# SebLague/Ray-Tracing

Hardware: AMD Instinct MI355X
Metric: Mrays/s at 1920x1080, 8 spp, 8 bounces; per-channel L2 vs reference (higher is better)
Workload: dtype f32

## Files before the change

### ray-tracing_amd/csrc/rt_context.hip

```cpp
#include <hip/hip_runtime.h>

#include <math.h>
#include <stdarg.h>
#include <stdio.h>
#include <stdlib.h>
#include <string.h>
#include <dlfcn.h>
#include <sys/mman.h>

#include <cmath>
#include <string>
#include <vector>

#include <algorithm>
#include <chrono>
#include <mutex>

#include "rt_kernels.h"
#include "../../include/rt_cost.h"
#include "../../include/rt_primary.h"
#include "../../include/rt_tile_cand.h"
#include "../../include/rt_aov.h"
#include "../../include/rt_denoise.h"
#include "../../include/rt_reproject.h"
#include "../../include/rt_variance.h"
#include "../../include/rt_adaptive.h"
#include "../../include/rt_motion.h"
#include "../../include/rt_query.h"
#include "../../include/rt_radiance.h"

#include "rt_denoise_launch.h"
#include "rt_denoise_math.h"
#include "rt_reproject_launch.h"
#include "rt_variance_launch.h"
#include "rt_adaptive_launch.h"
#include "rt_query_launch.h"
#include "rt_radiance_launch.h"
#include "rt_layout.h"
#include "rt_launch_order.h"
#include "rt_launch_plan.h"
#include "rt_scene_prep.h"
#include "rt_primary.h"
#include "rt_tile_cand.h"
#define RT_VERSION_STRING "raytrace_hip gfx950 abi=1"

static thread_local char g_err[512] = "";

struct RtContext;
struct LaunchJob;
struct HipOrder final : rt_order::Backend {
    RtContext* ctx = nullptr;
    hipEvent_t ev[rt_order::EVENT_COUNT] = {};
    LaunchJob* job = nullptr;
    hipStream_t stream(int s) const;
    int record(rt_order::Event e, int s) override;
    int wait(int s, rt_order::Event e) override;
    int sort(int s, int target) override;
    int trace(int s, int part, int parts) override;
    int accumulate(int s) override;
};

struct RtContext {
    int device = 0;
    hipStream_t ownStream = nullptr;
    hipStream_t stream = nullptr;
    hipStream_t sideStream = nullptr;
// ... 25 lines not shown
    DChunk* dChunks = nullptr;
    int nChunks = 0, nFiltered = 0, extWords = 0;
    float filterMaxOrigin = 0.0f;
    std::vector<RtBVHNode> hRootChildren;
    std::vector<RtSphere> hSpheres;
    int nSpheres = 0, nModels = 0, nTris = 0, nPairs = 0;
    bool flatScene = false;
    int stackEntries = 1;
    int wavesPerGroup = 1;
    uint32_t hotUnits = 0;
    uint32_t poolSpinLimit = 1u << 16;
    int poolMinItems = 4;
    int poolWaves = 1, poolCells = 0;
    uint32_t travLimit = 1u << 20;
    bool haveScene = false;
    std::vector<RtModel> hModels;
    std::vector<uint32_t> hRootCodes;
    std::vector<int32_t> hTriBase;
    PrimaryTris primaryTris;
    bool primaryOn = true;
    int lastPrimaryOn = -1;
    bool tileCandOn = true;
    int lastTileCand = -1;
    uint32_t* dTileCand[2] = {nullptr, nullptr};
    int tileCandTiles = 0;
    bool tileCandValid[2] = {false, false};
    TileCandKey tileCandKey[2];
    bool tileCandWanted = false;
    TileCandKey tileCandWant;

    RtParams params;
    bool haveParams = false;
    int frame = 1;

    unsigned long long* dCounters = nullptr;
    unsigned long long* dTileQueue = nullptr;
    unsigned long long tileQueueNext[2] = {0, 0};
    uint32_t* dTileCost = nullptr;
    uint32_t* dTileOrder[2] = {nullptr, nullptr};
    uint32_t* dTileKey = nullptr;
    int orderTiles = 0;
    int numCUs = 256;
    int occPerCU[16] = {0};
    size_t occBytes[16] = {0};
    bool verbose = false;
    void* dPxCold = nullptr;
    long long pxColdWaves = 0;
    int frameGroupOverride = 0;
    bool coalesce = true;
    int pending = 0;
    bool fuseFrames = true;
    int fuseCap = RT_FUSE_MIN;
// ... 261 lines not shown
        ctx->numCUs = prop.multiProcessorCount;
        HIP_TRY(ctx, hipStreamCreateWithFlags(&ctx->ownStream, hipStreamNonBlocking));
        ctx->stream = ctx->ownStream;
        HIP_TRY(ctx, hipMalloc(&ctx->dCounters, sizeof(unsigned long long) * RT_COUNTER_SLOTS * RT_COUNTER_FIELDS));
        HIP_TRY(ctx, hipMemsetAsync(ctx->dCounters, 0, sizeof(unsigned long long) * RT_COUNTER_SLOTS * RT_COUNTER_FIELDS, ctx->ownStream));
        HIP_TRY(ctx, hipStreamCreateWithFlags(&ctx->sideStream, hipStreamNonBlocking));
        HIP_TRY(ctx, hipMalloc(&ctx->dTileQueue, 2 * sizeof(unsigned long long)));
        HIP_TRY(ctx, hipMemsetAsync(ctx->dTileQueue, 0, 2 * sizeof(unsigned long long), ctx->ownStream));
        HIP_TRY(ctx, hipStreamSynchronize(ctx->ownStream));
        HIP_TRY(ctx, hipEventCreate(&ctx->evStart));
        HIP_TRY(ctx, hipEventCreate(&ctx->evStop));
        for (hipEvent_t& ev : ctx->backend.ev) HIP_TRY(ctx, hipEventCreateWithFlags(&ev, hipEventDisableTiming));
        return RT_OK;
    };
    if (int rc = init()) {
        rt_destroy(ctx);
        return rc;
    }
    memset(&ctx->params, 0, sizeof(ctx->params));
    if (const char* g = getenv("RT_GRID")) ctx->gridOverride = atoi(g);
    if (const char* g = getenv("RT_POOL_MIN_ITEMS")) ctx->poolMinItems = atoi(g);
    if (const char* g = getenv("RT_PRIMARY")) ctx->primaryOn = atoi(g) != 0;
    if (const char* g = getenv("RT_TILE_CAND")) ctx->tileCandOn = atoi(g) != 0;
    if (const char* g = getenv("RT_POOL_FAULT")) { if (atoi(g)) ctx->poolSpinLimit = 64u | 0x80000000u; }
    if (getenv("RT_VERBOSE")) ctx->verbose = true;
    if (const char* f = getenv("RT_FUSE_FRAMES")) ctx->fuseFrames = atoi(f) != 0;
    if (const char* l = getenv("RT_LPT")) ctx->order.lpt = atoi(l) != 0;
    if (const char* t = getenv("RT_TWO_STREAMS")) ctx->twoStreams = atoi(t) != 0;
    if (const char* c = getenv("RT_COALESCE")) ctx->coalesce = atoi(c) != 0;
    if (const char* fg = getenv("RT_FRAME_GROUP")) ctx->frameGroupOverride = atoi(fg);
    if (const char* al = getenv("RT_ALTERNATE")) ctx->order.alternate = ctx->alternateWanted = atoi(al) != 0;
    ctx->order.set_two_streams(ctx->twoStreams && ctx->sideStream);
    if (const char* fc = getenv("RT_FUSE_CAP"))
        if (const int cap = rt_plan::pinned_fuse_cap(atoi(fc))) { ctx->fuseCap = cap; ctx->fuseCapPinned = true; }
    *out = ctx;
    return RT_OK;
}

static void free_scene(RtContext* ctx)
{
    hipFree(ctx->dSpheres); ctx->dSpheres = nullptr;
    hipFree(ctx->dMaterials); ctx->dMaterials = nullptr;
    hipFree(ctx->dModels); ctx->dModels = nullptr;
    hipFree(ctx->dPairs); ctx->dPairs = nullptr;
    hipFree(ctx->dTris); ctx->dTris = nullptr;
    hipFree(ctx->dNorms); ctx->dNorms = nullptr;
// ... 228 lines not shown
    if (!ps.lay.arena && (rc = commit_vec(ctx, &ctx->dTris, ps.lay.triBuf, peer ? &peer->dTris : nullptr, peer))) return rc;
    if ((rc = commit_vec(ctx, &ctx->dNorms, ps.lay.normBuf, peer ? &peer->dNorms : nullptr, peer))) return rc;
    if (ps.lay.unitTri.size() && (rc = commit_vec(ctx, &ctx->dUnitTri, ps.lay.unitTri, peer ? &peer->dUnitTri : nullptr, peer))) return rc;
    if ((rc = commit_vec(ctx, &ctx->dBigLeaves, ps.lay.bigLeaves, peer ? &peer->dBigLeaves : nullptr, peer))) return rc;
    ctx->arenaLayout = ps.lay.arena;
    ctx->layoutUsed = ps.lay.used.name();
    if ((rc = commit_vec(ctx, &ctx->dFilters, ps.filters, peer ? &peer->dFilters : nullptr, peer))) return rc;
    if ((rc = commit_vec(ctx, &ctx->dChunks, ps.chunks, peer ? &peer->dChunks : nullptr, peer))) return rc;
    ctx->nChunks = (int)ps.chunks.size();
    ctx->nFiltered = ps.nFiltered;
    ctx->extWords = ps.extWords;
    ctx->filterMaxOrigin = ps.maxOrigin;
    ctx->sphereBound = ps.sphereBound;
    ctx->hRootChildren = ps.rootChildren;
    ctx->hSpheres = ps.hSpheres;
    ctx->nSpheres = (int)ps.hSpheres.size();
    ctx->nModels = (int)ps.hModels.size();
    ctx->nTris = ps.nTris;
    ctx->nPairs = (int)ps.nPairs;
    ctx->hTriBase = ps.lay.triBase;
    {
        const auto& triSpace = ps.lay.arena ? ps.lay.pairBuf : ps.lay.triBuf;
        primary_collect_tris(ps.flat, ps.dmodels.data(), (int)ps.dmodels.size(), triSpace.data(), triSpace.size(), ps.lay.bigLeaves.data(), ps.lay.bigLeaves.size(), ctx->primaryTris);
    }
    ctx->stackEntries = ps.flat ? 0 : ps.maxHeight;
    ctx->flatScene = ps.flat;
    ctx->hotUnits = ps.flat ? 0u : ps.lay.hotUnits;
    {
        const unsigned long long steps = (unsigned long long)ps.hModels.size() * (2ull * ps.nPairs + 2ull) + 16ull;
        const unsigned long long lim = 2ull * 64ull * steps;
        ctx->travLimit = lim > 0x7fffffffull ? 0x7fffffffu : (uint32_t)lim;
        if (const char* e = getenv("RT_TRAV_LIMIT")) ctx->travLimit = (uint32_t)strtoul(e, nullptr, 10);
    }
    ctx->wavesPerGroup = ctx->hotUnits ? ps.wavesPerGroup : 1;
    {
        int on = 1, waves = RT_MAX_WAVES_PER_GROUP_FLAT;
        if (const char* e = getenv("RT_POOL")) on = atoi(e);
        if (const char* e = getenv("RT_POOL_WAVES")) waves = atoi(e);
        if (waves < 1) waves = 1;
        if (waves > RT_MAX_WAVES_PER_GROUP_FLAT) waves = RT_MAX_WAVES_PER_GROUP_FLAT;
        const bool pooled = ps.flat && on;
        ctx->poolWaves = pooled ? waves : 1;
        ctx->poolCells = pooled ? (int)RT_POOL_CELLS : 0;
    }
    ctx->hModels = ps.hModels;
    ctx->hRootCodes = ps.rootCodes;
// ... 224 lines not shown
    memcpy(a.dirToSun, p.dirToSun, 12);
    memcpy(a.viewParams, p.viewParams, 12);
    memcpy(a.cam, p.camLocalToWorld, 64);
    a.rcpWm1 = rt_rcp((float)a.W - 1.0f);
    a.rcpHm1 = rt_rcp((float)a.H - 1.0f);
    a.rcpW = rt_rcp((float)a.W);
    a.rcpSpp = rt_rcp((float)a.spp);
    {
        bool fin = true;
        for (int k = 0; k < 16; k++) fin = fin && std::isfinite(a.cam[k]);
        const rt_f3 o = primary_cam_origin(a.cam);
        const bool noNegZero = rt_f2u(o.x) != 0x80000000u && rt_f2u(o.y) != 0x80000000u && rt_f2u(o.z) != 0x80000000u;
        a.raygenNoDefocus = (a.defocus == 0.0f && fin && noNegZero && std::isfinite(a.rcpW)) ? 1 : 0;
        const bool allowed = withTable && ctx->haveScene &&
                             primary_allowed(ctx->primaryOn, a.raygenNoDefocus != 0, ctx->flatScene, ctx->nSpheres, ctx->nModels, ctx->primaryTris);
        std::vector<float> sph;
        DModel dm[RT_PRIMARY_MAX_MODELS];
        if (allowed) {
            float bound;
            pack_spheres(ctx->hSpheres.data(), ctx->nSpheres, sph, &bound);
            for (int i = 0; i < ctx->nModels; i++) pack_model(ctx->hModels[i], ctx->hRootCodes[i], ctx->hTriBase[i], dm[i]);
        }
        primary_fill(a.primary, allowed, o, sph.data(), ctx->nSpheres, ctx->sphereBound, dm, ctx->nModels, ctx->primaryTris);
        if (withTable) {
            ctx->lastPrimaryOn = a.primary.on;
            ctx->lastTileCand = 0;
            ctx->tileCandWanted = ctx->tileCandOn && a.primary.on != 0;
            if (ctx->tileCandWanted) {
                TileCandKey& k = ctx->tileCandWant;
                tile_cand_key_init(k);
                memcpy(k.cam, a.cam, sizeof(k.cam));
                memcpy(k.viewParams, a.viewParams, sizeof(k.viewParams));
                k.rcpWm1 = a.rcpWm1; k.rcpHm1 = a.rcpHm1; k.rcpW = a.rcpW; k.diverge = a.diverge;
                k.camOrigin[0] = o.x; k.camOrigin[1] = o.y; k.camOrigin[2] = o.z;
                k.W = (int32_t)a.W; k.H = (int32_t)a.H;
                k.tilesX = a.tilesX; k.tiles = a.tilesX * a.tilesY;
                k.stripRows = a.stripRows; k.partIndex = a.partIndex; k.partCount = a.partCount;
                k.nSpheres = ctx->nSpheres;
                memcpy(k.sph, sph.data(), sizeof(float) * 4 * (size_t)ctx->nSpheres);
            }
        }
    }
    a.counters = ctx->dCounters;
    a.travLimit = ctx->travLimit;
    a.poolSpinLimit = ctx->poolSpinLimit;
    a.wavesPerGroup = 1;
}

}

struct LaunchPlan {
// ... 77 lines not shown
        hipFree(ctx->dTileKey); ctx->dTileKey = nullptr;
        HIP_TRY(ctx, hipMalloc(&ctx->dTileCost, sizeof(uint32_t) * tiles));
        HIP_TRY(ctx, hipMalloc(&ctx->dTileOrder[0], sizeof(uint32_t) * tiles));
        HIP_TRY(ctx, hipMalloc(&ctx->dTileOrder[1], sizeof(uint32_t) * tiles));
        HIP_TRY(ctx, hipMalloc(&ctx->dTileKey, sizeof(uint32_t) * tiles));
        HIP_TRY(ctx, hipMemsetAsync(ctx->dTileCost, 0, sizeof(uint32_t) * tiles, joined(ctx)));
        ctx->orderTiles = tiles;
        ctx->order.forget_order();
    }
    a.tileCost = ctx->dTileCost;
    return RT_OK;
}

static int prepare_tile_cand(RtContext* ctx, int tiles)
{
    if (!ctx->tileCandWanted || ctx->tileCandTiles == tiles) return RT_OK;
    HIP_TRY(ctx, hipStreamSynchronize(joined(ctx)));
    ctx->tileCandTiles = 0;
    for (int s = 0; s < 2; s++) {
        hipFree(ctx->dTileCand[s]); ctx->dTileCand[s] = nullptr;
        ctx->tileCandValid[s] = false;
    }
    for (int s = 0; s < 2; s++)
        if (hipMalloc(&ctx->dTileCand[s], sizeof(uint32_t) * (size_t)tiles) != hipSuccess) {
            (void)hipGetLastError();
            ctx->dTileCand[s] = nullptr;
            ctx->tileCandWanted = false;
            return RT_OK;
        }
    ctx->tileCandTiles = tiles;
    return RT_OK;
}

static_assert(sizeof(float4) == RT_STAGED_PIXEL_BYTES, "a staged colour is one float4");
static int prepare_staging(RtContext* ctx, KArgs& a, int nFrames, size_t nPix, int lane, bool split, bool* unavailable)
{
    *unavailable = false;
    const size_t need = (size_t)nFrames * nPix * RT_STAGED_PIXEL_BYTES;
    if (!ctx->stagingUnavailable && ctx->stagingBytes[lane] < need) {
        HIP_TRY(ctx, hipStreamSynchronize(joined(ctx)));
        for (int sl = 0; sl < (split && ctx->order.alternate ? 2 : 1); sl++) {
            const int b = sl == 0 ? lane : 1 - lane;
            if (ctx->stagingBytes[b] >= need) continue;
            hipFree(ctx->dStaging[b]);
            ctx->dStaging[b] = nullptr;
            ctx->stagingBytes[b] = 0;
            size_t slabBudget = RT_FUSE_SLAB_BYTES;
// ... 134 lines not shown
    w.flat = ctx->flatScene;
    w.spp = ctx->params.numRaysPerPixel;
    w.frameGroupOverride = ctx->frameGroupOverride;
    w.gridOverride = ctx->gridOverride;
    w.residentGroups = plan.resident;
    w.wavesPerGroup = plan.shape.wavesPerGroup;
    const rt_plan::PartPlan pp = rt_plan::plan_part(w, p, parts, ctx->tileQueueNext[s]);
    a.tileOrder = ctx->order.orderValid ? ctx->dTileOrder[ctx->order.orderCur] : nullptr;
    a.frameGroup = pp.frameGroup;
    a.frameGroupShift = pp.frameGroupShift;
    a.frameGroups = pp.frameGroups;
    a.launchTiles = pp.partTiles;
    a.launchItems = (int)pp.items;
    a.orderOffset = p;
    a.orderStride = parts;
    a.queueStart = pp.queueStart;
    if (ctx->verbose) fprintf(stderr, "[raytrace_hip] launch variant=%d part=%d/%d tiles=%d grid=%d x %d waves perCU=%d lds=%zu\n", plan.shape.variant, p, parts, pp.partTiles, pp.grid, plan.shape.wavesPerGroup, ctx->occPerCU[plan.shape.variant], plan.shape.ldsBytes);
    hipStream_t st = stream(s);
    a.pxCold = (float4*)((char*)ctx->dPxCold + (size_t)s * ctx->pxColdWaves * RT_COLD_STRIDE_BYTES);
    a.tileQueue = ctx->dTileQueue + s;
    a.tileQueueBase = pp.tileQueueBase;
    a.tileCand = nullptr;
    if (ctx->tileCandWanted && ctx->tileCandTiles == job->tiles && ctx->tileCandWant.tiles == job->tiles) {
        if (!ctx->tileCandValid[s] || memcmp(&ctx->tileCandKey[s], &ctx->tileCandWant, sizeof(TileCandKey)) != 0) {
            ctx->tileCandValid[s] = false;
            hipLaunchKernelGGL(rtk::rt_tile_cand_kernel, dim3((unsigned)((job->tiles + 255) / 256)), dim3(256), 0, st, ctx->tileCandWant, ctx->dTileCand[s]);
            HIP_TRY(ctx, hipGetLastError());
            ctx->tileCandKey[s] = ctx->tileCandWant;
            ctx->tileCandValid[s] = true;
        }
        a.tileCand = ctx->dTileCand[s];
        ctx->lastTileCand = 1;
    }
    RtContext::Tuner::Probe* probe = job->probe;
    const int fuseSlot = nFrames > 1 ? mark_fused_launch_begin(ctx, st) : -1;
    if (probe) hipEventRecord(probe->start, st);
    hipLaunchKernelGGL(parts == 2 ? plan.kernHalf : plan.kern, dim3(pp.grid), dim3(plan.shape.blockThreads), plan.shape.ldsBytes, st, a);
    if (probe) { hipEventRecord(probe->stop, st); probe->live = true; }
    HIP_TRY(ctx, hipGetLastError());
    mark_fused_launch_end(ctx, fuseSlot, st, nFrames);
    ctx->tileQueueNext[s] = pp.queueNext;
    return RT_OK;
}

int HipOrder::accumulate(int s)
{
    int blocks = (int)((job->nPix + 255) / 256);
    if (blocks > 4096) blocks = 4096;
    hipLaunchKernelGGL(rtk::rt_accumulate_kernel, dim3(blocks), dim3(256), 0, stream(s), (const float4*)ctx->dStaging[s], job->nFrames, job->nPix,
                       (float4*)job->a.accumulated, (float4*)job->a.frameRender, job->nPix);
    HIP_TRY(ctx, hipGetLastError());
    return RT_OK;
}

static int launch_frames(RtContext* ctx, int frame0, int nFrames)
// ... 275 lines not shown

int rt_debug_phase_profile(RtContext* ctx, uint64_t* out, int n)
{
    if (!ctx || !out || n < 2 * RT_N_PHASES) return fail(ctx, RT_ERR_INVALID_ARG, "rt_debug_phase_profile: need %d entries", 2 * RT_N_PHASES);
    RT_FLUSH(ctx);
    std::vector<unsigned long long> h;
    if (int rc = read_counter_block(ctx, h)) return rc;
    for (int f = 0; f < 2 * RT_N_PHASES; f++) out[f] = sum_field(h, 8 + f);
    if (n > 2 * RT_N_PHASES) out[2 * RT_N_PHASES] = sum_field(h, 6);
    for (int p = 0; p < RT_N_PHASES && 2 * RT_N_PHASES + 1 + p < n; p++) out[2 * RT_N_PHASES + 1 + p] = p < 3 ? sum_field(h, 8 + 2 * RT_N_PHASES + p) : 0;
    return RT_OK;
}

struct DevScratch {
    void* p = nullptr;
    ~DevScratch() { if (p) hipFree(p); }
    hipError_t alloc(size_t bytes) { return hipMalloc(&p, bytes); }
    float* f() const { return (float*)p; }
};

int rt_debug_fused_frames_cap(const RtContext* ctx) { return ctx ? ctx->fuseCap : RT_ERR_INVALID_ARG; }
int rt_debug_primary_table(const RtContext* ctx) { return ctx ? ctx->lastPrimaryOn : RT_ERR_INVALID_ARG; }
int rt_debug_tile_cand(const RtContext* ctx) { return ctx ? ctx->lastTileCand : RT_ERR_INVALID_ARG; }

int rt_debug_intersect(RtContext* ctx, const float* origins, const float* dirs, int n, float* out10)
{
    if (ctx) RT_FLUSH(ctx);
    if (!ctx) return fail(nullptr, RT_ERR_INVALID_ARG, "null context");
    if (!ctx->haveScene) return fail(ctx, RT_ERR_STATE, "rt_debug_intersect before rt_upload_scene");
    if (n < 0 || (n && (!origins || !dirs || !out10))) return fail(ctx, RT_ERR_INVALID_ARG, "rt_debug_intersect: bad arguments");
    if (n == 0) return RT_OK;
    HIP_TRY(ctx, hipSetDevice(ctx->device));
    DevScratch dO, dD, dR;
    HIP_TRY(ctx, dO.alloc((size_t)n * 12));
    HIP_TRY(ctx, dD.alloc((size_t)n * 12));
    HIP_TRY(ctx, dR.alloc((size_t)n * 40));
    HIP_TRY(ctx, hipMemcpy(dO.p, origins, (size_t)n * 12, hipMemcpyHostToDevice));
    HIP_TRY(ctx, hipMemcpy(dD.p, dirs, (size_t)n * 12, hipMemcpyHostToDevice));
    KArgs a;
    fill_args(ctx, 1, 1, a);
    hipLaunchKernelGGL(rtk::rt_debug_intersect_kernel, dim3((n + RT_WAVE - 1) / RT_WAVE), dim3(RT_WAVE), 0, joined(ctx), a, dO.f(), dD.f(), n, dR.f());
    HIP_TRY(ctx, hipGetLastError());
    HIP_TRY(ctx, hipStreamSynchronize(joined(ctx)));
    HIP_TRY(ctx, hipMemcpy(out10, dR.p, (size_t)n * 40, hipMemcpyDeviceToHost));
    return RT_OK;
}
// ... 1696 lines not shown
```

### ray-tracing_amd/csrc/rt_device.h

```cpp
#ifndef RT_DEVICE_H
#define RT_DEVICE_H

#include "rt_records.h"
#include "rt_primary.h"

struct KArgs {
    const float* spheres;
    const float* sphereQuick;
    float sphereBound;
    const DMaterial* materials;
    const DModel* models;
    const DPair* pairs;
    const DTri* tris;
    const DTriN* norms;
    const uint32_t* bigLeaves;
    const DFilter* filters;
    const float* filterPairs;
    float filterMaxOrigin;
    int32_t nSpheres, nModels;
    const DChunk* chunks;
    int32_t nChunks, nFiltered, extWords;
    float* frameRender;
    float* accumulated;
    uint32_t W, H;
// ... 9 lines not shown
    float cam[16];
    float rcpWm1, rcpHm1;
    float rcpW;
    float rcpSpp;
    int32_t suspendNum;
    int32_t raygenNoDefocus;
    unsigned long long* counters;
    int32_t launchTiles, orderOffset, orderStride;
    int32_t launchItems;
    float4* pxCold;
    int32_t frameGroup;
    int32_t frameGroups;
    float* staging;
    uint32_t stagingStride;
    int32_t queueStart;
    unsigned long long* tileQueue;
    unsigned long long tileQueueBase;
    const uint32_t* tileOrder;
    uint32_t* tileCost;
    int32_t poolCells;
    int32_t frameGroupShift;
    uint32_t poolSpinLimit;
    PrimaryTable primary;
    const uint32_t* tileCand;
};

#endif
```

### ray-tracing_amd/csrc/rt_kernels.h

```cpp
#ifndef RT_KERNELS_H
#define RT_KERNELS_H

#include <hip/hip_runtime.h>

#include "../../include/rt_abi.h"
#include "../../include/rt_math.h"
#include "rt_device.h"
#include "rt_tile_cand.h"

#ifndef RT_SUSPEND_NUM
#define RT_SUSPEND_NUM 3
#define RT_SUSPEND_DEN 8
#endif
#ifndef RT_INNER_BURST
#define RT_INNER_BURST 3
#endif

namespace rtk {

#define RT_CAS __attribute__((address_space(4)))
#define RT_LDS __attribute__((address_space(3)))

__device__ __forceinline__ float hw_min(float a, float b) { return __builtin_fminf(a, b); }
__device__ __forceinline__ float hw_max(float a, float b) { return __builtin_fmaxf(a, b); }

__device__ __forceinline__ float box_dst(rt_f3 pos, rt_f3 invDir, const float* bmin, const float* bmax)
{
    float tminx = (bmin[0] - pos.x) * invDir.x, tmaxx = (bmax[0] - pos.x) * invDir.x;
    float tminy = (bmin[1] - pos.y) * invDir.y, tmaxy = (bmax[1] - pos.y) * invDir.y;
    float tminz = (bmin[2] - pos.z) * invDir.z, tmaxz = (bmax[2] - pos.z) * invDir.z;
    float tNear = hw_max(hw_max(hw_min(tminx, tmaxx), hw_min(tminy, tmaxy)), hw_min(tminz, tmaxz));
// ... 132 lines not shown
    bool didHit = keep && dst > 0 && u >= 0 && v >= 0 && w >= 0;
    if (didHit && dst < bestDst) {
        bestDst = dst;
        bestTri = triUnit;
        bu = u;
        bv = v;
        bdet = determinant;
    }
}

struct Trav {
    unsigned long long cand;
    int m;
    uint32_t cur;
    int sp;
    bool rootStep;
    rt_f3 lpos, ldir, linv;
    int triBase;
    bool cull;
};

template <bool STATS, bool FLAT, bool MANY, bool ANY = false, bool PRIMARY = false>
__device__ __forceinline__ void begin_intersect(const KArgs& a, rt_f3 rpos, rt_f3 rdir, uint32_t* extBase, SceneHit& h, Trav& t, Stats& st, const float tmax = 0.0f,
                                                const RT_CAS PrimaryTable* pt = nullptr, const uint32_t* tileCand = nullptr, const uint32_t tile = 0u)
{
    h.dst = RT_INF;
    h.obj = -1;
    h.tri = -1;
    h.u = h.v = h.det = 0.0f;
    h.backface = false;

    const RT_CAS float* sph = (const RT_CAS float*)a.spheres;
    const RT_CAS float* sphq = (const RT_CAS float*)a.sphereQuick;
    const float qa = rt_dot(rdir, rdir);
    const float od = __builtin_fmaf(rpos.x, rdir.x, __builtin_fmaf(rpos.y, rdir.y, rpos.z * rdir.z));
    const float oo = PRIMARY ? 0.0f : __builtin_fmaf(rpos.x, rpos.x, __builtin_fmaf(rpos.y, rpos.y, rpos.z * rpos.z));
    const float negMargin = -(7.62939453125e-06f * qa * (PRIMARY ? pt->ooBound : oo + a.sphereBound));
    typedef float rt_f2v __attribute__((ext_vector_type(2)));
    const rt_f2v dx2 = {rdir.x, rdir.x}, dy2 = {rdir.y, rdir.y}, dz2 = {rdir.z, rdir.z};
    const rt_f2v ox2 = {rpos.x, rpos.x}, oy2 = {rpos.y, rpos.y}, oz2 = {rpos.z, rpos.z};
    const rt_f2v od2 = {od, od}, oo2 = {oo, oo}, qa2 = {qa, qa}, m2 = {-2.0f, -2.0f};
    for (int base = 0; base < a.nSpheres; base += 32) {
        const int n = (a.nSpheres - base) < 32 ? (a.nSpheres - base) : 32;
        uint32_t cand = 0;
        if (PRIMARY && tileCand != nullptr) {
            cand = tileCand[tile];
            if (STATS) {
                for (uint32_t rest = ~cand & (n >= 32 ? 0xffffffffu : (1u << n) - 1u); rest; rest &= rest - 1) {
                    const int s = base + __builtin_ctz(rest);
                    const rt_f3 off = rt_v3(pt->sph[s][0], pt->sph[s][1], pt->sph[s][2]);
                    const float qb = 2 * rt_dot(off, rdir);
                    const float disc = qb * qb - 4 * qa * pt->sph[s][3];
                    if (disc >= 0 && (-qb + rt_sqrt(disc)) * rt_rcp(2 * qa) >= 0) st.filterViolations++;
                }
            }
        } else
        for (int k = 0; k < n; k += 2) {
            const RT_CAS float* q = PRIMARY ? &pt->pair[0][0] + 4 * (base + k) : sphq + 4 * (base + k);
            const rt_f2v cx = {q[0], q[1]}, cy = {q[2], q[3]}, cz = {q[4], q[5]}, kk = {q[6], q[7]};
            const rt_f2v cd = __builtin_elementwise_fma(cx, dx2, __builtin_elementwise_fma(cy, dy2, cz * dz2));
            const rt_f2v b = od2 - cd;
            rt_f2v ct = kk;
            if (!PRIMARY) {
                const rt_f2v co = __builtin_elementwise_fma(cx, ox2, __builtin_elementwise_fma(cy, oy2, cz * oz2));
                ct = __builtin_elementwise_fma(m2, co, oo2) + kk;
            }
            const rt_f2v dq = __builtin_elementwise_fma(b, b, -(qa2 * ct));
            const bool keep0 = !(dq.x < negMargin);
            const bool keep1 = (k + 1 < n) && !(dq.y < negMargin);
// ... 304 lines not shown
                    h.obj = a.nSpheres + t.m;
                    h.backface = h.det < 0;
                    if (ANY && h.dst < tmax) break;
                }
            }
            if (ANY && h.dst < tmax) {
                t.cur = RT_CODE_DONE;
                t.sp = 0;
                t.cand = 0;
            } else if (t.sp == 0) t.cur = RT_CODE_NEXT_MODEL;
            else t.cur = stackBase[(--t.sp) * RT_WAVE];
        }
        if (++watchdog > a.travLimit) {
            t.cur = RT_CODE_DONE; t.sp = 0; t.cand = 0;
            if ((int)(threadIdx.x & 63) == __ffsll((long long)__ballot(1)) - 1) atomicAdd(a.counters + 7, 1ull);
        }
        RT_TRAV_VOTE();
    } while ((nA + nB + nC) * RT_SUSPEND_DEN > enteredNum);
#undef RT_TRAV_VOTE
    return t.cur == RT_CODE_DONE;
}

template <bool STATS, bool ANY = false, bool PRIMARY = false>
__device__ __forceinline__ void traverse_flat(const KArgs& a, rt_f3 rpos, rt_f3 rdir, SceneHit& h, Stats& st, const float tmax = 0.0f, const RT_CAS PrimaryTable* pt = nullptr)
{
    const RT_CAS DModel* cm = (const RT_CAS DModel*)a.models;
    const DTri* __restrict__ tris = a.tris;
    const RT_CAS float* pr = PRIMARY ? &pt->tri[0][0] : nullptr;
    for (int m = 0; m < a.nModels; m++) {
        if (ANY && __ballot(!(h.dst < tmax)) == 0ull) break;
        const RT_CAS DModel& M = cm[m];
        rt_f3 lpos;
        if (PRIMARY) lpos = rt_v3(pt->lpos[m][0], pt->lpos[m][1], pt->lpos[m][2]);
        else lpos = rt_v3(M.w2l[0] * rpos.x + M.w2l[1] * rpos.y + M.w2l[2] * rpos.z + M.w2l[3] * 1.0f,
                          M.w2l[4] * rpos.x + M.w2l[5] * rpos.y + M.w2l[6] * rpos.z + M.w2l[7] * 1.0f,
                          M.w2l[8] * rpos.x + M.w2l[9] * rpos.y + M.w2l[10] * rpos.z + M.w2l[11] * 1.0f);
        rt_f3 ldir = rt_v3(M.w2l[0] * rdir.x + M.w2l[1] * rdir.y + M.w2l[2] * rdir.z + M.w2l[3] * 0.0f,
                           M.w2l[4] * rdir.x + M.w2l[5] * rdir.y + M.w2l[6] * rdir.z + M.w2l[7] * 0.0f,
                           M.w2l[8] * rdir.x + M.w2l[9] * rdir.y + M.w2l[10] * rdir.z + M.w2l[11] * 0.0f);
        const uint32_t code = M.rootCode;
        uint32_t count = (code >> 24) & 0x7fu;
        uint32_t start = code & RT_CODE_MAX_INLINE_START;
        if (count == 0) {
            count = a.bigLeaves[2 * start + 1];
            start = a.bigLeaves[2 * start];
        }
        if (STATS) { st.leaf++; st.tri += count; }
        const int first = M.triBase + (int)start;
        const bool cull = M.cullBackface != 0;
        for (uint32_t i = 0; i < count; i++) {
            phase_mark<STATS>(st, PH_TRI);
            if (ANY && h.dst < tmax) break;
            const float before = h.dst;
            tri_test<PRIMARY>(tris, first + 3 * (int)i, lpos, ldir, cull, h.dst, h.tri, h.u, h.v, h.det, pr);
            if (PRIMARY) pr += 4;
            if (h.dst < before) {
                h.obj = a.nSpheres + m;
                h.backface = h.det < 0;
            }
        }
    }
}

template <bool STATS>
__device__ __forceinline__ void intersect_scene(const KArgs& a, rt_f3 rpos, rt_f3 rdir, uint32_t* stackBase, uint32_t* extBase, SceneHit& h, Stats& st)
{
    Trav t;
    if (a.nChunks) {
        begin_intersect<STATS, false, true>(a, rpos, rdir, extBase, h, t, st);
        traverse<STATS, false, true>(a, rpos, rdir, stackBase, extBase, h, t, st, (const RT_LDS char*)nullptr, 0u);
    } else {
        begin_intersect<STATS, false, false>(a, rpos, rdir, extBase, h, t, st);
        traverse<STATS, false, false>(a, rpos, rdir, stackBase, extBase, h, t, st, (const RT_LDS char*)nullptr, 0u);
    }
}
// ... 381 lines not shown
                    rt_f3 jfp = focusPoint + camRight * (jj.x * c.diverge * invNumPixelsX) + camUp * (jj.y * c.diverge * invNumPixelsX);
                    rpos = rayOrigin;
                    rdir = rt_normalize(jfp - rayOrigin);
                    transmittance = rt_v3s(1.0f);
                    pathLight = rt_v3s(0.0f);
                    if (MANY) extBase[(1 + a.extWords) * RT_WAVE] = 0u;
                    else bounce = 0;
                    PXU(PX_SAMPLE) = grouped ? (PXU(PX_SAMPLE) & 0xffff0000u) | (uint32_t)(sample + 1) : (uint32_t)(sample + 1);
                    if (c.maxBounce >= 0) pathActive = true;
                    else { PXF(PX_TIX) = PXF(PX_TIX) + 0.0f; PXF(PX_TIY) = PXF(PX_TIY) + 0.0f; PXF(PX_TIZ) = PXF(PX_TIZ) + 0.0f; }
                    if constexpr (COST) if (pathActive) {
                        uint4* const o = RT_COST_SLOT(c) + 1;
                        uint4 p = *o;
                        p.x -= st.inner; p.y -= st.leaf; p.z -= st.tri;
                        *o = p;
                    }
                }
            }
            if (pathActive) {
                phase_mark<STATS>(st, PH_SPHERES);
                if constexpr (FLAT && !MANY && !COST) {
                    const RT_CAS PrimaryTable* const pt = &cold_args().primary;
                    if (pt->on != 0 && __ballot(bounce != 0) == 0ull) {
                        const uint32_t* const tileCand = cold_args().tileCand;
                        const uint32_t tile = tileCand ? __float_as_uint(PX_COLD(cold_args())[RT_WAVE].w) : 0u;
                        begin_intersect<STATS, FLAT, MANY, false, true>(a, rpos, rdir, extBase, h, t, st, 0.0f, pt, tileCand, tile);
                        traverse_flat<STATS, false, true>(a, rpos, rdir, h, st, 0.0f, pt);
                    } else {
                        begin_intersect<STATS, FLAT, MANY>(a, rpos, rdir, extBase, h, t, st);
                        traverse_flat<STATS>(a, rpos, rdir, h, st);
                    }
                    segments++;
                    inTrav = true;
                } else {
                    begin_intersect<STATS, FLAT, MANY>(a, rpos, rdir, extBase, h, t, st);
                    segments++;
                    inTrav = true;
                    if (FLAT) traverse_flat<STATS>(a, rpos, rdir, h, st);
                }
            }
        }
        if constexpr (!POOL) {
#include "rt_shade_phase.inl"
        }
        }
        if constexpr (POOL) {
            pool_exchange<STATS>(a, s_lds, lane, pxu, PX_COLD(cold_args()), laneDone, pathActive, inTrav, rpos, rdir, transmittance, pathLight, rng, bounce, h, segments, st);
            if (!laneDone) {
#include "rt_shade_phase.inl"
            }
// ... 325 lines not shown
    case 7: r = rt_smoothstep(0.0f, y[i], x[i]); break;
    }
    out[i] = r;
}

__global__ void __launch_bounds__(1024) rt_order_kernel(const uint32_t* cost, uint32_t* key, uint32_t* order, int nTiles)
{
    __shared__ uint32_t hist[1024];
    __shared__ uint32_t base[1024];
    const int t = threadIdx.x;
    hist[t] = 0;
    for (int i = t; i < nTiles; i += 1024) key[i] = 1023u - (cost[i] < 1023u ? cost[i] : 1023u);
    __syncthreads();
    for (int i = t; i < nTiles; i += 1024) atomicAdd(&hist[key[i]], 1u);
    __syncthreads();
    if (t == 0) {
        uint32_t run = 0;
        for (int k = 0; k < 1024; k++) { base[k] = run; run += hist[k]; }
    }
    __syncthreads();
    for (int i = t; i < nTiles; i += 1024) order[atomicAdd(&base[key[i]], 1u)] = (uint32_t)i;
}

__global__ void __launch_bounds__(256) rt_tile_cand_kernel(const TileCandKey k, uint32_t* out)
{
    const int tile = (int)(blockIdx.x * 256u + threadIdx.x);
    if (tile >= k.tiles) return;
    int x0, y0;
    tile_cand_origin(k, tile, &x0, &y0);
    out[tile] = tile_cand_mask(k, x0, y0);
}

__global__ void rt_display_kernel(const float4* src, float4* dst, size_t n, int frame)
{
    const float inv = rt_rcp((float)frame);
    size_t i = (size_t)blockIdx.x * blockDim.x + threadIdx.x;
    const size_t stride = (size_t)gridDim.x * blockDim.x;
    for (; i < n; i += stride) {
        float4 v = src[i];
        dst[i] = make_float4(v.x * inv, v.y * inv, v.z * inv, v.w * inv);
    }
}
__global__ void rt_display_srgb8_kernel(const float4* src, uint32_t* dst, int width, int rows, int frame, int flipY)
{
    const float inv = rt_rcp((float)frame);
    const size_t n = (size_t)width * rows;
    size_t i = (size_t)blockIdx.x * blockDim.x + threadIdx.x;
    const size_t stride = (size_t)gridDim.x * blockDim.x;
    for (; i < n; i += stride) {
        float4 v = src[i];
        uint32_t r = rt_srgb8(v.x * inv), g = rt_srgb8(v.y * inv), b = rt_srgb8(v.z * inv);
        size_t row = i / width, col = i - row * width;
        size_t o = flipY ? ((size_t)(rows - 1) - row) * width + col : i;
// ... 45 lines not shown
```

### ray-tracing_amd/hip.py

```python
import ctypes as C
import os

import numpy as np

from . import abi

_HERE = os.path.dirname(os.path.abspath(__file__))
LIB_PATH = os.environ.get("RT_HIP_LIB") or os.path.join(_HERE, "lib", "libraytrace_hip.so")

ABI_SYMBOLS = [
    "rt_create", "rt_destroy", "rt_last_error", "rt_set_stream", "rt_resize", "rt_set_partition", "rt_local_rows",
    "rt_local_to_global_row", "rt_bind_render_targets", "rt_get_render_targets", "rt_upload_scene", "rt_update_models",
    "rt_update_spheres", "rt_set_params", "rt_reset_accumulation", "rt_render_frame", "rt_render_frames",
    "rt_synchronize", "rt_get_frame", "rt_read_frame", "rt_read_accumulated", "rt_display", "rt_display_srgb8",
    "rt_write_accumulated", "rt_timer_begin", "rt_timer_end",
    "rt_enable_stats", "rt_reset_counters", "rt_get_counters", "rt_build_bvh", "rt_build_bvh_mt", "rt_build_bvh_gpu", "rt_build_bvh_gpu_release", "rt_camera_view_params", "rt_version",
    "rt_debug_intersect", "rt_debug_math_eval", "rt_debug_phase_profile", "rt_build_bvh_gpu_batch",
    "rt_flush", "rt_validate_scene", "rt_debug_layout", "rt_debug_layout_free", "rt_debug_fused_frames_cap",
    "rt_create_multi", "rt_destroy_multi", "rt_multi_count", "rt_multi_context", "rt_multi_resize", "rt_multi_upload_scene",
    "rt_multi_update_models", "rt_multi_update_spheres", "rt_multi_set_params", "rt_multi_reset_accumulation",
    "rt_multi_render_frame", "rt_multi_render_frames", "rt_multi_synchronize", "rt_gather_accumulated", "rt_gather_frame",
    "rt_multi_get_counters", "rt_multi_last_gather_ms", "rt_multi_peer_access", "rt_gather_accumulated_to_device", "rt_gather_frame_to_device",
    "rt_gather_rccl",
]
COST_SYMBOLS = ["rt_render_cost"]
PRIMARY_SYMBOLS = ["rt_debug_primary_table"]
TILE_CAND_SYMBOLS = ["rt_debug_tile_cand"]
AOV_SYMBOLS = ["rt_render_aov", "rt_render_aov_to_device"]
DENOISE_SYMBOLS = ["rt_denoise_default_params", "rt_denoise_buffers", "rt_denoise", "rt_denoise_to_device"]
REPROJECT_SYMBOLS = ["rt_reproject_default_params", "rt_reproject_buffers", "rt_reproject_accumulated", "rt_resolve_buffers", "rt_resolve",
                     "rt_resolve_to_device"]
MOTION_SYMBOLS = ["rt_render_aov_centre", "rt_render_aov_centre_to_device", "rt_motion_from_scene", "rt_reproject_buffers_moving",
                  "rt_reproject_accumulated_moving"]
VARIANCE_SYMBOLS = ["rt_denoise_variance_default_params", "rt_moments_update_buffers", "rt_denoise_variance_buffers", "rt_variance_update",
                    "rt_variance_reset", "rt_variance_carry", "rt_variance_read_moments", "rt_variance_moments_to_device", "rt_denoise_variance",
                    "rt_denoise_variance_to_device"]
ADAPTIVE_SYMBOLS = ["rt_adaptive_default_params", "rt_adaptive_select_buffers", "rt_adaptive_select", "rt_adaptive_set_tiles", "rt_adaptive_read_tiles",
                    "rt_adaptive_read_tile_error", "rt_adaptive_render_frames"]
QUERY_SYMBOLS = ["rt_query_closest", "rt_query_closest_buffers", "rt_query_occluded", "rt_query_occluded_buffers"]
RADIANCE_SYMBOLS = ["rt_radiance_trace", "rt_radiance_trace_buffers"]
COST_FIELDS = ("segments", "innerSteps", "leafSteps", "triTests", "primaryInnerSteps", "primaryLeafSteps", "primaryTriTests", "firstHit")


class HipApi(abi.CApi):
    _EXTRA = {
        "create": (C.c_int, [C.c_int, C.POINTER(C.c_void_p)]),
        "set_stream": (C.c_int, [C.c_void_p, C.c_void_p]),
        "set_partition": (C.c_int, [C.c_void_p, C.c_int, C.c_int, C.c_int]),
        "local_rows": (C.c_int, [C.c_void_p]),
        "local_to_global_row": (C.c_int, [C.c_void_p, C.c_int]),
# ... 418 lines not shown
        self._check(self.api.bind_render_targets(self.h, frame_ptr, accum_ptr))

    def render_targets(self):
        f, a = C.c_void_p(), C.c_void_p()
        self._check(self.api.get_render_targets(self.h, C.byref(f), C.byref(a)))
        return f.value, a.value

    def gather_rccl(self, nccl_comm, root, device_ptr, nbytes, accumulated=True):
        self._check(self.api.gather_rccl(self.h, nccl_comm, int(root), 1 if accumulated else 0, device_ptr, nbytes))

    def fused_frames_cap(self):
        return self.api.debug_fused_frames_cap(self.h)

    def primary_table(self):
        fn = self.api.lib.rt_debug_primary_table
        fn.restype, fn.argtypes = C.c_int, [C.c_void_p]
        return fn(self.h)

    def tile_cand(self):
        fn = self.api.lib.rt_debug_tile_cand
        fn.restype, fn.argtypes = C.c_int, [C.c_void_p]
        return fn(self.h)

    def synchronize(self):
        self._check(self.api.synchronize(self.h))

    def flush(self):
        self._check(self.api.flush(self.h))

    def timer_begin(self):
        self._check(self.api.timer_begin(self.h))

    def timer_end(self):
        self._check(self.api.timer_end(self.h))

    def enable_stats(self, on=True):
        self._check(self.api.enable_stats(self.h, 1 if on else 0))

    def debug_intersect(self, origins, dirs):
        o = np.ascontiguousarray(origins, dtype=np.float32).reshape(-1, 3)
        d = np.ascontiguousarray(dirs, dtype=np.float32).reshape(-1, 3)
        out = np.zeros((len(o), 10), dtype=np.float32)
        self._check(self.api.debug_intersect(self.h, o.ctypes.data, d.ctypes.data, len(o), out.ctypes.data))
        return out

    PHASES = ["loop", "raygen", "spheres", "traverse_call", "model", "inner", "tri", "shade_hit", "sky", "sphere_roots", "glass", "refill"]
# ... 197 lines not shown
```

Measured before the change: 53000.

## Add per-tile conservative triangle culling for primary rays in flat scenes

```diff
diff --git a/include/rt_tile_tri.h b/include/rt_tile_tri.h
--- /dev/null
+++ b/include/rt_tile_tri.h
@@ -0,0 +1,16 @@
+#ifndef RT_TILE_TRI_ABI_H
+#define RT_TILE_TRI_ABI_H
+
+#include "rt_abi.h"
+
+#ifdef __cplusplus
+extern "C" {
+#endif
+
+int rt_debug_tile_tri(const RtContext* ctx);
+
+#ifdef __cplusplus
+}
+#endif
+
+#endif
diff --git a/ray-tracing_amd/csrc/rt_context.hip b/ray-tracing_amd/csrc/rt_context.hip
--- a/ray-tracing_amd/csrc/rt_context.hip
+++ b/ray-tracing_amd/csrc/rt_context.hip
@@ -20,6 +20,7 @@
 #include "../../include/rt_cost.h"
 #include "../../include/rt_primary.h"
 #include "../../include/rt_tile_cand.h"
+#include "../../include/rt_tile_tri.h"
 #include "../../include/rt_aov.h"
 #include "../../include/rt_denoise.h"
 #include "../../include/rt_reproject.h"
@@ -42,6 +43,7 @@
 #include "rt_scene_prep.h"
 #include "rt_primary.h"
 #include "rt_tile_cand.h"
+#include "rt_tile_tri.h"
 #define RT_VERSION_STRING "raytrace_hip gfx950 abi=1"
 
 static thread_local char g_err[512] = "";
@@ -113,12 +115,17 @@
     int lastPrimaryOn = -1;
     bool tileCandOn = true;
     int lastTileCand = -1;
-    uint32_t* dTileCand[2] = {nullptr, nullptr};
+    uint2* dTileCand[2] = {nullptr, nullptr};
     int tileCandTiles = 0;
     bool tileCandValid[2] = {false, false};
     TileCandKey tileCandKey[2];
     bool tileCandWanted = false;
     TileCandKey tileCandWant;
+    bool tileTriOn = true;
+    int lastTileTri = -1;
+    TileTris tileTris;
+    TileTriKey tileTriKey[2];
+    TileTriKey tileTriWant;
 
     RtParams params;
     bool haveParams = false;
@@ -426,6 +433,7 @@
     if (const char* g = getenv("RT_POOL_MIN_ITEMS")) ctx->poolMinItems = atoi(g);
     if (const char* g = getenv("RT_PRIMARY")) ctx->primaryOn = atoi(g) != 0;
     if (const char* g = getenv("RT_TILE_CAND")) ctx->tileCandOn = atoi(g) != 0;
+    if (const char* g = getenv("RT_TILE_TRI")) ctx->tileTriOn = atoi(g) != 0;
     if (const char* g = getenv("RT_POOL_FAULT")) { if (atoi(g)) ctx->poolSpinLimit = 64u | 0x80000000u; }
     if (getenv("RT_VERBOSE")) ctx->verbose = true;
     if (const char* f = getenv("RT_FUSE_FRAMES")) ctx->fuseFrames = atoi(f) != 0;
@@ -700,6 +708,7 @@
     {
         const auto& triSpace = ps.lay.arena ? ps.lay.pairBuf : ps.lay.triBuf;
         primary_collect_tris(ps.flat, ps.dmodels.data(), (int)ps.dmodels.size(), triSpace.data(), triSpace.size(), ps.lay.bigLeaves.data(), ps.lay.bigLeaves.size(), ctx->primaryTris);
+        tile_tri_collect(ps.flat, ps.dmodels.data(), (int)ps.dmodels.size(), triSpace.data(), triSpace.size(), ps.lay.bigLeaves.data(), ps.lay.bigLeaves.size(), ctx->tileTris);
     }
     ctx->stackEntries = ps.flat ? 0 : ps.maxHeight;
     ctx->flatScene = ps.flat;
@@ -970,11 +979,14 @@
             for (int i = 0; i < ctx->nModels; i++) pack_model(ctx->hModels[i], ctx->hRootCodes[i], ctx->hTriBase[i], dm[i]);
         }
         primary_fill(a.primary, allowed, o, sph.data(), ctx->nSpheres, ctx->sphereBound, dm, ctx->nModels, ctx->primaryTris);
+        a.triEnds = a.primary.on ? tile_tri_ends(ctx->primaryTris.count, ctx->nModels) : 0u;
         if (withTable) {
             ctx->lastPrimaryOn = a.primary.on;
             ctx->lastTileCand = 0;
+            ctx->lastTileTri = 0;
             ctx->tileCandWanted = ctx->tileCandOn && a.primary.on != 0;
             if (ctx->tileCandWanted) {
+                tile_tri_key_fill(ctx->tileTriWant, ctx->tileTriOn, ctx->tileTris, dm, ctx->nModels, a.primary.lpos);
                 TileCandKey& k = ctx->tileCandWant;
                 tile_cand_key_init(k);
                 memcpy(k.cam, a.cam, sizeof(k.cam));
@@ -1098,7 +1110,7 @@
         ctx->tileCandValid[s] = false;
     }
     for (int s = 0; s < 2; s++)
-        if (hipMalloc(&ctx->dTileCand[s], sizeof(uint32_t) * (size_t)tiles) != hipSuccess) {
+        if (hipMalloc(&ctx->dTileCand[s], sizeof(uint2) * (size_t)tiles) != hipSuccess) {
             (void)hipGetLastError();
             ctx->dTileCand[s] = nullptr;
             ctx->tileCandWanted = false;
@@ -1279,15 +1291,18 @@
     a.tileQueueBase = pp.tileQueueBase;
     a.tileCand = nullptr;
     if (ctx->tileCandWanted && ctx->tileCandTiles == job->tiles && ctx->tileCandWant.tiles == job->tiles) {
-        if (!ctx->tileCandValid[s] || memcmp(&ctx->tileCandKey[s], &ctx->tileCandWant, sizeof(TileCandKey)) != 0) {
+        if (!ctx->tileCandValid[s] || memcmp(&ctx->tileCandKey[s], &ctx->tileCandWant, sizeof(TileCandKey)) != 0 ||
+            memcmp(&ctx->tileTriKey[s], &ctx->tileTriWant, sizeof(TileTriKey)) != 0) {
             ctx->tileCandValid[s] = false;
-            hipLaunchKernelGGL(rtk::rt_tile_cand_kernel, dim3((unsigned)((job->tiles + 255) / 256)), dim3(256), 0, st, ctx->tileCandWant, ctx->dTileCand[s]);
+            hipLaunchKernelGGL(rtk::rt_tile_cand_kernel, dim3((unsigned)((job->tiles + 255) / 256)), dim3(256), 0, st, ctx->tileCandWant, ctx->tileTriWant, ctx->dTileCand[s]);
             HIP_TRY(ctx, hipGetLastError());
             ctx->tileCandKey[s] = ctx->tileCandWant;
+            ctx->tileTriKey[s] = ctx->tileTriWant;
             ctx->tileCandValid[s] = true;
         }
         a.tileCand = ctx->dTileCand[s];
         ctx->lastTileCand = 1;
+        ctx->lastTileTri = ctx->tileTriWant.on;
     }
     RtContext::Tuner::Probe* probe = job->probe;
     const int fuseSlot = nFrames > 1 ? mark_fused_launch_begin(ctx, st) : -1;
@@ -1609,6 +1624,7 @@
 int rt_debug_fused_frames_cap(const RtContext* ctx) { return ctx ? ctx->fuseCap : RT_ERR_INVALID_ARG; }
 int rt_debug_primary_table(const RtContext* ctx) { return ctx ? ctx->lastPrimaryOn : RT_ERR_INVALID_ARG; }
 int rt_debug_tile_cand(const RtContext* ctx) { return ctx ? ctx->lastTileCand : RT_ERR_INVALID_ARG; }
+int rt_debug_tile_tri(const RtContext* ctx) { return ctx ? ctx->lastTileTri : RT_ERR_INVALID_ARG; }
 
 int rt_debug_intersect(RtContext* ctx, const float* origins, const float* dirs, int n, float* out10)
 {
diff --git a/ray-tracing_amd/csrc/rt_device.h b/ray-tracing_amd/csrc/rt_device.h
--- a/ray-tracing_amd/csrc/rt_device.h
+++ b/ray-tracing_amd/csrc/rt_device.h
@@ -55,7 +55,8 @@
     int32_t frameGroupShift;
     uint32_t poolSpinLimit;
     PrimaryTable primary;
-    const uint32_t* tileCand;
+    const uint2* tileCand;
+    uint32_t triEnds;
 };
 
 #endif
diff --git a/ray-tracing_amd/csrc/rt_kernels.h b/ray-tracing_amd/csrc/rt_kernels.h
--- a/ray-tracing_amd/csrc/rt_kernels.h
+++ b/ray-tracing_amd/csrc/rt_kernels.h
@@ -7,6 +7,7 @@
 #include "../../include/rt_math.h"
 #include "rt_device.h"
 #include "rt_tile_cand.h"
+#include "rt_tile_tri.h"
 
 #ifndef RT_SUSPEND_NUM
 #define RT_SUSPEND_NUM 3
@@ -185,7 +186,8 @@
 
 template <bool STATS, bool FLAT, bool MANY, bool ANY = false, bool PRIMARY = false>
 __device__ __forceinline__ void begin_intersect(const KArgs& a, rt_f3 rpos, rt_f3 rdir, uint32_t* extBase, SceneHit& h, Trav& t, Stats& st, const float tmax = 0.0f,
-                                                const RT_CAS PrimaryTable* pt = nullptr, const uint32_t* tileCand = nullptr, const uint32_t tile = 0u)
+                                                const RT_CAS PrimaryTable* pt = nullptr, const uint2* tileCand = nullptr, const uint32_t tile = 0u,
+                                                uint32_t* triUnion = nullptr, uint32_t* triLane = nullptr)
 {
     h.dst = RT_INF;
     h.obj = -1;
@@ -203,11 +205,24 @@
     const rt_f2v dx2 = {rdir.x, rdir.x}, dy2 = {rdir.y, rdir.y}, dz2 = {rdir.z, rdir.z};
     const rt_f2v ox2 = {rpos.x, rpos.x}, oy2 = {rpos.y, rpos.y}, oz2 = {rpos.z, rpos.z};
     const rt_f2v od2 = {od, od}, oo2 = {oo, oo}, qa2 = {qa, qa}, m2 = {-2.0f, -2.0f};
+    uint32_t tileSph = 0;
+    if (PRIMARY && tileCand != nullptr) {
+        const uint2 rec = tileCand[tile];
+        tileSph = rec.x;
+        uint32_t uni = 0;
+        for (unsigned long long rest = __ballot(1); rest;) {
+            const uint32_t w = (uint32_t)__builtin_amdgcn_readlane((int)rec.y, __builtin_ctzll(rest));
+            uni |= w;
+            rest &= ~__ballot(rec.y == w);
+        }
+        *triUnion = uni;
+        if (STATS) *triLane = rec.y;
+    }
     for (int base = 0; base < a.nSpheres; base += 32) {
         const int n = (a.nSpheres - base) < 32 ? (a.nSpheres - base) : 32;
         uint32_t cand = 0;
         if (PRIMARY && tileCand != nullptr) {
-            cand = tileCand[tile];
+            cand = tileSph;
             if (STATS) {
                 for (uint32_t rest = ~cand & (n >= 32 ? 0xffffffffu : (1u << n) - 1u); rest; rest &= rest - 1) {
                     const int s = base + __builtin_ctz(rest);
@@ -558,13 +573,24 @@
 }
 
 template <bool STATS, bool ANY = false, bool PRIMARY = false>
-__device__ __forceinline__ void traverse_flat(const KArgs& a, rt_f3 rpos, rt_f3 rdir, SceneHit& h, Stats& st, const float tmax = 0.0f, const RT_CAS PrimaryTable* pt = nullptr)
+__device__ __forceinline__ void traverse_flat(const KArgs& a, rt_f3 rpos, rt_f3 rdir, SceneHit& h, Stats& st, const float tmax = 0.0f, const RT_CAS PrimaryTable* pt = nullptr,
+                                              const uint32_t triUnion = 0xffffffffu, const uint32_t triEnds = 0u, const uint32_t triLane = 0xffffffffu)
 {
     const RT_CAS DModel* cm = (const RT_CAS DModel*)a.models;
     const DTri* __restrict__ tris = a.tris;
     const RT_CAS float* pr = PRIMARY ? &pt->tri[0][0] : nullptr;
+    uint32_t k0 = 0;
     for (int m = 0; m < a.nModels; m++) {
         if (ANY && __ballot(!(h.dst < tmax)) == 0ull) break;
+        uint32_t live = 0xffffffffu, laneBits = 0xffffffffu;
+        if (PRIMARY) {
+            const uint32_t k1 = (triEnds >> (8 * m)) & 0xffu;
+            live = (triUnion >> k0) & ((1u << (k1 - k0)) - 1u);
+            if (STATS) laneBits = triLane >> k0;
+            pr = &pt->tri[0][0] + 4 * k0;
+            k0 = k1;
+            if (!STATS && live == 0u) continue;
+        }
         const RT_CAS DModel& M = cm[m];
         rt_f3 lpos;
         if (PRIMARY) lpos = rt_v3(pt->lpos[m][0], pt->lpos[m][1], pt->lpos[m][2]);
@@ -587,6 +613,13 @@
         for (uint32_t i = 0; i < count; i++) {
             phase_mark<STATS>(st, PH_TRI);
             if (ANY && h.dst < tmax) break;
+            if (PRIMARY && STATS && !((laneBits >> i) & 1u)) {
+                float best = RT_INF, bu, bv, bdet;
+                int btri = -1;
+                tri_test<PRIMARY>(tris, first + 3 * (int)i, lpos, ldir, cull, best, btri, bu, bv, bdet, pr);
+                if (btri >= 0) st.filterViolations++;
+            }
+            if (PRIMARY && !((live >> i) & 1u)) { pr += 4; continue; }
             const float before = h.dst;
             tri_test<PRIMARY>(tris, first + 3 * (int)i, lpos, ldir, cull, h.dst, h.tri, h.u, h.v, h.det, pr);
             if (PRIMARY) pr += 4;
@@ -1014,10 +1047,11 @@
                 if constexpr (FLAT && !MANY && !COST) {
                     const RT_CAS PrimaryTable* const pt = &cold_args().primary;
                     if (pt->on != 0 && __ballot(bounce != 0) == 0ull) {
-                        const uint32_t* const tileCand = cold_args().tileCand;
+                        const uint2* const tileCand = cold_args().tileCand;
                         const uint32_t tile = tileCand ? __float_as_uint(PX_COLD(cold_args())[RT_WAVE].w) : 0u;
-                        begin_intersect<STATS, FLAT, MANY, false, true>(a, rpos, rdir, extBase, h, t, st, 0.0f, pt, tileCand, tile);
-                        traverse_flat<STATS, false, true>(a, rpos, rdir, h, st, 0.0f, pt);
+                        uint32_t triUnion = 0xffffffffu, triLane = 0xffffffffu;
+                        begin_intersect<STATS, FLAT, MANY, false, true>(a, rpos, rdir, extBase, h, t, st, 0.0f, pt, tileCand, tile, &triUnion, &triLane);
+                        traverse_flat<STATS, false, true>(a, rpos, rdir, h, st, 0.0f, pt, triUnion, cold_args().triEnds, triLane);
                     } else {
                         begin_intersect<STATS, FLAT, MANY>(a, rpos, rdir, extBase, h, t, st);
                         traverse_flat<STATS>(a, rpos, rdir, h, st);
@@ -1389,13 +1423,13 @@
     for (int i = t; i < nTiles; i += 1024) order[atomicAdd(&base[key[i]], 1u)] = (uint32_t)i;
 }
 
-__global__ void __launch_bounds__(256) rt_tile_cand_kernel(const TileCandKey k, uint32_t* out)
+__global__ void __launch_bounds__(256) rt_tile_cand_kernel(const TileCandKey k, const TileTriKey kt, uint2* out)
 {
     const int tile = (int)(blockIdx.x * 256u + threadIdx.x);
     if (tile >= k.tiles) return;
     int x0, y0;
     tile_cand_origin(k, tile, &x0, &y0);
-    out[tile] = tile_cand_mask(k, x0, y0);
+    out[tile] = make_uint2(tile_cand_mask(k, x0, y0), tile_tri_mask(k, kt, x0, y0));
 }
 
 __global__ void rt_display_kernel(const float4* src, float4* dst, size_t n, int frame)
diff --git a/ray-tracing_amd/csrc/rt_tile_tri.h b/ray-tracing_amd/csrc/rt_tile_tri.h
--- /dev/null
+++ b/ray-tracing_amd/csrc/rt_tile_tri.h
@@ -0,0 +1,177 @@
+#ifndef RT_TILE_TRI_H
+#define RT_TILE_TRI_H
+
+#include <stdint.h>
+#include <string.h>
+
+#include "../../include/rt_math.h"
+#include "rt_records.h"
+#include "rt_tile_cand.h"
+
+#define RT_TILE_TRI_MAX_MODELS 4
+#define RT_TILE_TRI_MAX_TRIS 16
+
+struct TileTris {
+    bool usable = false;
+    int nModels = 0;
+    int count[RT_TILE_TRI_MAX_MODELS] = {0, 0, 0, 0};
+    float a[RT_TILE_TRI_MAX_TRIS][3];
+    float ab[RT_TILE_TRI_MAX_TRIS][3];
+    float ac[RT_TILE_TRI_MAX_TRIS][3];
+};
+
+static inline void tile_tri_collect(bool flat, const DModel* models, int nModels, const unsigned char* triSpace, size_t triSpaceBytes,
+                                    const uint32_t* bigLeaves, size_t nBigLeafWords, TileTris& out)
+{
+    out = TileTris();
+    if (!flat || nModels < 0 || nModels > RT_TILE_TRI_MAX_MODELS) return;
+    int total = 0;
+    for (int m = 0; m < nModels; m++) {
+        const uint32_t code = models[m].rootCode;
+        uint32_t count = (code >> 24) & 0x7fu, start = code & RT_CODE_MAX_INLINE_START;
+        if (count == 0) {
+            if (2 * (size_t)start + 1 >= nBigLeafWords) return;
+            count = bigLeaves[2 * (size_t)start + 1];
+            start = bigLeaves[2 * (size_t)start];
+        }
+        if (count > (uint32_t)(RT_TILE_TRI_MAX_TRIS - total)) return;
+        for (uint32_t i = 0; i < count; i++) {
+            const long long unit = (long long)models[m].triBase + (long long)start + 3ll * (long long)i;
+            if (unit < 0 || ((size_t)unit + 3) * 16 > triSpaceBytes) return;
+            DTri t;
+            memcpy(&t, triSpace + (size_t)unit * 16, sizeof(t));
+            float q[12];
+            memcpy(q, &t, sizeof(q));
+            for (int d = 0; d < 3; d++) { out.a[total][d] = q[d]; out.ab[total][d] = q[3 + d]; out.ac[total][d] = q[6 + d]; }
+            total++;
+        }
+        out.count[m] = (int)count;
+    }
+    out.nModels = nModels;
+    out.usable = true;
+}
+
+struct TileTriKey {
+    int32_t on;
+    int32_t nModels;
+    int32_t count[RT_TILE_TRI_MAX_MODELS];
+    int32_t pad[2];
+    float m3[RT_TILE_TRI_MAX_MODELS][9];
+    float lpos[RT_TILE_TRI_MAX_MODELS][3];
+    float p0[RT_TILE_TRI_MAX_TRIS][3];
+    float ab[RT_TILE_TRI_MAX_TRIS][3];
+    float ac[RT_TILE_TRI_MAX_TRIS][3];
+};
+
+static inline void tile_tri_key_init(TileTriKey& k) { memset(&k, 0, sizeof(k)); }
+
+static inline void tile_tri_key_fill(TileTriKey& k, bool on, const TileTris& tris, const DModel* models, int nModels, const float (*lpos)[4])
+{
+    tile_tri_key_init(k);
+    if (!on || !tris.usable || tris.nModels != nModels) return;
+    k.on = 1;
+    k.nModels = nModels;
+    int t = 0;
+    for (int m = 0; m < nModels; m++) {
+        k.count[m] = tris.count[m];
+        for (int r = 0; r < 3; r++)
+            for (int c = 0; c < 3; c++) k.m3[m][3 * r + c] = models[m].w2l[4 * r + c];
+        for (int d = 0; d < 3; d++) k.lpos[m][d] = lpos[m][d];
+        for (int i = 0; i < tris.count[m]; i++, t++)
+            for (int d = 0; d < 3; d++) {
+                k.p0[t][d] = tris.a[t][d] - lpos[m][d];
+                k.ab[t][d] = tris.ab[t][d];
+                k.ac[t][d] = tris.ac[t][d];
+            }
+    }
+}
+
+static inline uint32_t tile_tri_ends(const int* count, int nModels)
+{
+    uint32_t ends = 0, run = 0;
+    for (int m = 0; m < RT_TILE_TRI_MAX_MODELS; m++) {
+        if (m < nModels) run += (uint32_t)count[m];
+        ends |= (run & 0xffu) << (8 * m);
+    }
+    return ends;
+}
+
+RT_HD float tile_tri_len(rt_f3 v) { return rt_sqrt(rt_dot(v, v)); }
+
+RT_HD uint32_t tile_tri_mask(const TileCandKey& k, const TileTriKey& kt, int x0, int y0)
+{
+    if (!kt.on) return 0xffffffffu;
+    int total = 0;
+    for (int m = 0; m < kt.nModels && m < RT_TILE_TRI_MAX_MODELS; m++) total += kt.count[m];
+    if (total > RT_TILE_TRI_MAX_TRIS) total = RT_TILE_TRI_MAX_TRIS;
+    const uint32_t all = (1u << (total > 0 ? total : 0)) - 1u;
+    const rt_f3 o = rt_v3(k.camOrigin[0], k.camOrigin[1], k.camOrigin[2]);
+    const rt_f3 R = rt_v3(k.cam[0], k.cam[1], k.cam[2]), U = rt_v3(k.cam[4], k.cam[5], k.cam[6]), F = rt_v3(k.cam[8], k.cam[9], k.cam[10]);
+    const float fx = (((float)x0 + 3.5f) * k.rcpWm1 - 0.5f) * k.viewParams[0];
+    const float fy = (((float)y0 + 3.5f) * k.rcpHm1 - 0.5f) * k.viewParams[1];
+    const float jit = rt_abs(k.diverge * k.rcpW);
+    const float ex = 1.01f * (4.0f * rt_abs(k.rcpWm1 * k.viewParams[0]) + jit), ey = 1.01f * (4.0f * rt_abs(k.rcpHm1 * k.viewParams[1]) + jit);
+    const rt_f3 Fz = F * k.viewParams[2];
+    rt_f3 cw[4];
+    float g[4], maxLen = 0.0f;
+    for (int i = 0; i < 4; i++) {
+        cw[i] = R * (fx + ((i & 1) ? ex : -ex)) + U * (fy + ((i & 2) ? ey : -ey)) + Fz;
+        g[i] = tile_tri_len(cw[i]);
+        if (!(tile_cand_finite(g[i]) && g[i] > 1e-30f && rt_dot(cw[i], Fz) > 0.0f)) return all;
+        maxLen = rt_max(maxLen, g[i]);
+    }
+    const float epsW = 3.814697265625e-06f * (2.0f * tile_tri_len(o) + maxLen);
+    if (!tile_cand_finite(epsW)) return all;
+    for (int i = 0; i < 4; i++) g[i] += epsW;
+
+    uint32_t mask = 0;
+    int t = 0;
+    for (int m = 0; m < kt.nModels && m < RT_TILE_TRI_MAX_MODELS; m++) {
+        const float* w = kt.m3[m];
+        float normM = 0.0f;
+        for (int j = 0; j < 9; j++) normM += w[j] * w[j];
+        normM = rt_sqrt(normM);
+        rt_f3 c[4];
+        bool fin = tile_cand_finite(normM);
+        for (int i = 0; i < 4; i++) {
+            c[i] = rt_v3(w[0] * cw[i].x + w[1] * cw[i].y + w[2] * cw[i].z, w[3] * cw[i].x + w[4] * cw[i].y + w[5] * cw[i].z,
+                         w[6] * cw[i].x + w[7] * cw[i].y + w[8] * cw[i].z);
+            fin = fin && tile_cand_finite(c[i].x) && tile_cand_finite(c[i].y) && tile_cand_finite(c[i].z);
+        }
+        for (int i = 0; i < kt.count[m] && t < RT_TILE_TRI_MAX_TRIS; i++, t++) {
+            const rt_f3 V0 = rt_v3(kt.p0[t][0], kt.p0[t][1], kt.p0[t][2]);
+            const rt_f3 AB = rt_v3(kt.ab[t][0], kt.ab[t][1], kt.ab[t][2]), AC = rt_v3(kt.ac[t][0], kt.ac[t][1], kt.ac[t][2]);
+            const rt_f3 V1 = V0 + AB, V2 = V0 + AC;
+            const rt_f3 N = rt_cross(AB, AC);
+            const float lenN = tile_tri_len(N), lenAB = tile_tri_len(AB), lenAC = tile_tri_len(AC), lenP = tile_tri_len(V0);
+            const float S = lenP * (lenAB + lenAC) + lenAB * lenAC;
+            const float E = 1.52587890625e-05f * S;
+            const float s = rt_dot(V0, N);
+            bool drop = false;
+            const bool sound = fin && tile_cand_finite(S) && tile_cand_finite(lenN) && tile_cand_finite(s) &&
+                               lenN > 1e-5f * (lenAB * lenAC) && rt_abs(s) > 1e-4f * (lenP * lenN) &&
+                               lenP > 1e-15f && tile_tri_len(V1) > 1e-15f && tile_tri_len(V2) > 1e-15f &&
+                               lenAB > 1e-15f && lenAC > 1e-15f && S > 1e-30f;
+            if (sound) {
+                const float sg = s > 0.0f ? 1.0f : -1.0f;
+                const rt_f3 Va[3] = {V0, V1, V2}, Vb[3] = {V1, V2, V0};
+                for (int e = 0; e < 3 && !drop; e++) {
+                    const rt_f3 n = rt_cross(Va[e], Vb[e]) * sg;
+                    const float lenE = tile_tri_len(n);
+                    if (!tile_cand_finite(lenE)) continue;
+                    bool outside = true;
+                    for (int i = 0; i < 4; i++) {
+                        const float margin = normM * (g[i] * (E + 9.5367431640625e-07f * lenE) + lenE * epsW);
+                        const float d = rt_dot(n, c[i]);
+                        outside = outside && tile_cand_finite(margin) && tile_cand_finite(d) && d < -margin;
+                    }
+                    drop = outside;
+                }
+            }
+            if (!drop) mask |= 1u << t;
+        }
+    }
+    return mask;
+}
+
+#endif
diff --git a/ray-tracing_amd/hip.py b/ray-tracing_amd/hip.py
--- a/ray-tracing_amd/hip.py
+++ b/ray-tracing_amd/hip.py
@@ -26,6 +26,7 @@
 COST_SYMBOLS = ["rt_render_cost"]
 PRIMARY_SYMBOLS = ["rt_debug_primary_table"]
 TILE_CAND_SYMBOLS = ["rt_debug_tile_cand"]
+TILE_TRI_SYMBOLS = ["rt_debug_tile_tri"]
 AOV_SYMBOLS = ["rt_render_aov", "rt_render_aov_to_device"]
 DENOISE_SYMBOLS = ["rt_denoise_default_params", "rt_denoise_buffers", "rt_denoise", "rt_denoise_to_device"]
 REPROJECT_SYMBOLS = ["rt_reproject_default_params", "rt_reproject_buffers", "rt_reproject_accumulated", "rt_resolve_buffers", "rt_resolve",
@@ -490,6 +491,11 @@
         fn.restype, fn.argtypes = C.c_int, [C.c_void_p]
         return fn(self.h)
 
+    def tile_tri(self):
+        fn = self.api.lib.rt_debug_tile_tri
+        fn.restype, fn.argtypes = C.c_int, [C.c_void_p]
+        return fn(self.h)
+
     def synchronize(self):
         self._check(self.api.synchronize(self.h))
 
```

Result: no change. 53420 (median of 5 runs) (+0.8%).
